# zxhuang1698/ShapeClipper

Measured on AMD Instinct MI355X. Metric: train-step images/sec (Pix3D cfg, bs32/GPU), higher is better.
Workload: dtype f32 (bf16x3-split MFMA, fp32 accumulate)

## Files before the change

### include/shapeclipper_hip.h

```cpp
#ifndef SHAPECLIPPER_HIP_H
#define SHAPECLIPPER_HIP_H
#include <stdint.h>
#ifdef __cplusplus
extern "C" {
#endif

int sc_chamfer3d_forward(const float* xyz1, const float* xyz2, float* dist1, float* dist2,
                         int32_t* idx1, int32_t* idx2, int b, int n, int m, void* stream);

int sc_chamfer3d_forward_split(const float* xyz1, const float* xyz2, float* dist1, float* dist2,
                               int32_t* idx1, int32_t* idx2, int b, int n, int m, int nsplit,
                               void* workspace, void* stream);

long long sc_chamfer3d_grid_workspace_bytes(int b, int n, int m);
int sc_chamfer3d_forward_grid(const float* xyz1, const float* xyz2, float* dist1, float* dist2,
                              int32_t* idx1, int32_t* idx2, int b, int n, int m, void* workspace, void* stream);

int sc_chamfer3d_backward(const float* xyz1, const float* xyz2, float* gradxyz1, float* gradxyz2,
                          const float* graddist1, const float* graddist2, const int32_t* idx1,
                          const int32_t* idx2, int b, int n, int m, void* stream);

long long sc_chamfer3d_backward_ordered_workspace_bytes(int b, int n, int m);
int sc_chamfer3d_backward_ordered_chunk(void);
int sc_chamfer3d_backward_ordered(const float* xyz1, const float* xyz2, float* gradxyz1, float* gradxyz2,
// ... 272 lines not shown

int sc_marching_cubes_mesh_vertex_blocks_per_image(int n_axis);
int sc_marching_cubes_mesh_vertex_count(const float* level, int n_images, int n_axis, float iso, int* block_counts, void* stream);
int sc_marching_cubes_mesh_vertex_scan(const int* block_counts, int n_images, int n_axis, long long* block_offsets, long long* per_image,
                                       void* stream);
int sc_marching_cubes_mesh_vertex_emit(const float* level, int n_images, int n_axis, float iso, const long long* block_offsets, float* verts,
                                       int* vmap, void* stream);
int sc_marching_cubes_mesh_face_emit(int n_images, int n_axis, const long long* block_offsets, const unsigned char* masks, const int* vmap,
                                     int* faces, void* stream);

int sc_camera_rays_forward(const float* pose, const float* intr, const long long* ray_idx, int n_images,
                           int rays_per_image, int image_width, float* cam_loc, float* ray_dirs, float* depth_fac,
                           void* stream);
int sc_camera_rays_backward(const float* pose, const float* intr, const long long* ray_idx, int n_images,
                            int rays_per_image, int image_width, const float* g_cam_loc, const float* g_ray_dirs,
                            const float* g_depth_fac, float* g_pose, float* g_intr, void* stream);

int sc_pose_from_trig_forward(const float* azim, const float* elev, const float* theta, const float* scale_focal,
                              const float* scale_dist, int n_images, float cam_dist, float focal, int image_width,
                              int image_height, float* pose, float* intr, void* stream);
int sc_pose_from_trig_backward(const float* azim, const float* elev, const float* theta, const float* scale_focal,
                               const float* scale_dist, int n_images, float cam_dist, float focal, int image_width,
                               int image_height, const float* g_pose, const float* g_intr, float* g_azim,
                               float* g_elev, float* g_theta, float* g_scale_focal, float* g_scale_dist, void* stream);

int sc_estimator_head_forward(const float* trig, const float* size_lin, const float* persp_lin, int n_rows,
                              float size_range, float persp_range, float* azim, float* elev, float* theta,
                              float* scale_focal, float* scale_dist, void* stream);
int sc_estimator_head_backward(const float* trig, const float* size_lin, const float* persp_lin, int n_rows,
                               float size_range, float persp_range, const float* const* grads, int n_groups,
                               float* g_trig, float* g_size_lin, float* g_persp_lin, void* stream);

int sc_camera_prior_max_images(void);
int sc_camera_prior_forward(const float* azim, const float* elev, const float* theta, const float* flip_azim,
                            const float* flip_elev, const float* flip_theta, int n_images, float elev_lo, float elev_hi,
                            float theta_lo, float theta_hi, float margin_eps, int emd_p, float* out, float* grads,
                            void* stream);
int sc_camera_prior_backward(const float* grads, int n_images, const float* G_margin, const float* G_uniform,
                             const float* G_sym, float* g_azim, float* g_elev, float* g_theta, float* g_flip_azim,
                             float* g_flip_elev, float* g_flip_theta, void* stream);

int sc_transform_normal_forward(const float* normals, const float* pose, int n_images, int n_per_image, float* out,
                                void* stream);
int sc_transform_normal_backward(const float* normals, const float* g_out, int n_images, int n_per_image, float* g_pose,
                                 void* stream);

int sc_loss_total_forward(const float* const* values, const float* weights, int n_terms, float* total, unsigned char* bad,
                          void* stream);
int sc_loss_total_backward(const float* weights, int n_terms, const float* G, float* g_values, void* stream);

long long sc_conv3x3_pack_floats(int cin, int cout, int hw);
long long sc_conv3x3_workspace_floats(int hw);
int sc_conv3x3_tile_channels(int hw);
int sc_conv3x3_pack_multi(const long long* table, int n, float* dst, long long total, void* stream);
int sc_conv3x3_pack_multi_units(const long long* table, int n, float* dst, long long total, void* stream);
int sc_conv3x3_pack(const float* w, float* w_pack, int cin, int cout, int hw, int transpose_flip, void* stream);
int sc_conv3x3_forward(const float* x, const float* w_pack, float* out, float* workspace, int batch, int cin, int cout, int hw,
                       void* stream);

long long sc_conv3x3_pack_floats_split(int cin, int cout, int hw);
long long sc_conv3x3_workspace_floats_split(int hw);
int sc_conv3x3_tile_channels_split(int hw);
int sc_conv3x3_forward_split(const float* x, const float* w_pack, float* out, float* workspace, int batch, int cin, int cout, int hw,
                             void* stream);
int sc_conv3x3_forward_add(const float* x, const float* w_pack, const float* addend, float* out, float* workspace, int batch, int cin,
                           int cout, int hw, int split, void* stream);

long long sc_conv3x3s2_bd_pack_floats(int cin, int cout, int hw);
long long sc_conv3x3s2_bd_workspace_floats(int hw);
int sc_conv3x3s2_bd_pack(const float* w, float* w_pack, int cin, int cout, int hw, void* stream);
int sc_conv3x3s2_backward_data(const float* gy, const float* w_pack, float* gx, float* workspace, int batch, int cin, int cout, int hw,
                               void* stream);
int sc_conv3x3s2_wgrad(const float* gy, const float* x, float* dw, float* workspace, int batch, int cin, int cout, int hw, void* stream);
long long sc_conv3x3s2_pack_floats(int cin, int cout, int hw);
long long sc_conv3x3s2_workspace_floats(int hw);
int sc_conv3x3s2_forward(const float* x, const float* w_pack, float* out, float* workspace, int batch, int cin, int cout, int hw,
                         void* stream);

long long sc_conv3x3_wgrad_workspace_floats(int cin, int cout);
int sc_conv3x3_wgrad(const float* gy, const float* x, float* dw, float* workspace, int batch, int cin, int cout, int hw, void* stream);
int sc_conv3x3_wgrad_split(const float* gy, const float* x, float* dw, float* workspace, int batch, int cin, int cout, int hw, void* stream);

long long sc_conv_stem_wgrad_workspace_floats(void);
int sc_conv_stem_forward(const float* x, const float* w, float* out, int batch, void* stream);
int sc_conv_stem_wgrad(const float* gy, const float* x, float* dw, float* workspace, int batch, void* stream);

long long sc_conv1x1s2_wgrad_workspace_floats(int cin, int cout);
int sc_conv1x1s2_forward(const float* x, const float* w, float* out, int batch, int cin, int cout, int hin, void* stream);
int sc_conv1x1s2_backward_data(const float* gy, const float* w, float* gx, int batch, int cin, int cout, int hin, void* stream);
int sc_conv1x1s2_wgrad(const float* gy, const float* x, float* dw, float* workspace, int batch, int cin, int cout, int hin, void* stream);

typedef struct sc_block_args {
    const float *x, *pf1, *pf2, *pb1, *pb2;
    const float *g1, *b1, *g2, *b2;
    float *rm1, *rv1, *rm2, *rv2;
    int64_t *nt1, *nt2;
    float *y1, *a1, *y2, *out, *st1, *st2;
    float *conv_ws, *bn_ws, *wgrad_ws;
    const float* d_out;
    float *dy2, *dres, *da1, *dy1, *dx, *gw1, *gw2, *dgb1, *dgb2;
    int batch, channels, hw, groups, training, split, need_dx;
    float mom1, eps1, mom2, eps2;
} sc_block_args;
int sc_basic_block_forward(const sc_block_args* args, void* stream);
int sc_basic_block_backward(const sc_block_args* args, void* stream);

int sc_linear_bn_supported(int N, int Cin, int Cout, int groups);
int sc_linear_bn_forward(const float* x, const float* w, const float* gamma, const float* beta, const float* res, float* y, float* out,
                         float* save_mean, float* save_rstd, float* run_mean, float* run_var, int64_t* n_tracked, int N, int Cin,
                         int Cout, int groups, int training, int relu, float eps, float momentum, void* stream);
int sc_linear_bn_backward(const float* g_out, const float* gy_next, const float* w_next, const float* g_add, int Cnext, const float* out,
                          const float* y, const float* save_mean, const float* save_rstd, const float* gamma, const float* x, float* gy,
                          float* g_res, float* dw, float* dgamma, float* dbeta, int N, int Cin, int Cout, int groups, int training, int relu,
                          void* stream);
int sc_linear_backward_data(const float* gy, const float* w, const float* g_add, float* dx, int N, int Cin, int Cout, void* stream);

int sc_latent_bias_forward(const float* z, const float* lat, const float* bias, const float* post, float* out, int B, int Z, int L, int NL,
                           void* stream);
int sc_latent_bias_backward(const float* g, const float* z, const float* lat, const float* post, float* g_z, float* g_lat, float* g_bias,
                            int B, int Z, int L, int NL, void* stream);

int sc_silhouette_distance(const float* masks, int n, int H, int W, float* dist, void* stream);
int sc_silhouette_rays(const float* dist, int n, int H, int W, int n_rays, double uniform_fac, const long long* seeds,
                       long long* ray_idx, void* stream);

int sc_clip_preprocess(const unsigned char* rgba, int n, int H, int W, int n_px, int bg, const int* h_bounds, const int* h_coef,
                       int h_taps, const int* v_bounds, const int* v_coef, int v_taps, unsigned char* tmp, float* out, void* stream);

int sc_vis_frames(const float* x, long long n_pixels, int channels, int kind, float lo, float scale, unsigned char* out, void* stream);

int sc_rgb_points_forward_split(const float* points, const float* grad, const float* feat, const float* v_pack,
                                const float* dbias, int n_points, int n_per_image, int n_images, int symmetric,
                                float* rgb, float* normal, void* stream);

long long sc_level_largest_component_scratch_bytes(int n_images, int n_axis);
int sc_level_largest_component(const float* level, int n_images, int n_axis, float iso, float* level_out, int32_t* n_components,
                               int32_t* inside_voxels, int32_t* kept_voxels, void* scratch, void* stream);

#define SC_SURFACE_HIT_MAX_RAYS (1 << 30)
int sc_ray_first_crossing(const float* z_vals, const float* sdf, int n_rays, int n_samples, float iso, float* t_lo, float* t_hi,
                          float* f_lo, float* f_hi, int32_t* hit, void* stream);
int sc_ray_bracket_step(const float* cam_loc, const float* ray_dirs, const float* f_new, const float* t_prev, int n_rays, float iso,
                        float* t_lo, float* t_hi, float* f_lo, float* f_hi, const int32_t* hit, float* t, float* points, void* stream);

int sc_set_reserved_cus(int n);
int sc_grid_cus(void);
int sc_conv3x3_release_tables(void);

#ifdef __cplusplus
}
#endif
#endif
```

### shapeclipper_amd/csrc/conv_stem.hip

```cpp
#include <hip/hip_runtime.h>

#include "grid_cus.hpp"
#include "shapeclipper_hip.h"

namespace sc {

typedef float st_f32x16 __attribute__((ext_vector_type(16)));

constexpr int ST_WI = 224, ST_WO = 112, ST_WP = 230, ST_K = 147, ST_KP = 148, ST_CO = 64;
constexpr int ST_HWI = ST_WI * ST_WI, ST_HWO = ST_WO * ST_WO;
constexpr int SF_PT = 256;
constexpr int SF_ROWS = 13;
constexpr int SF_CH = SF_ROWS * ST_WP;
constexpr int SF_PATCH = 3 * SF_CH;
constexpr int SF_WLD = 96;
constexpr int SF_LDS = ST_KP * SF_WLD + SF_PATCH;
constexpr int SF_NLOAD = (3 * SF_ROWS + 7) / 8;

__global__ __launch_bounds__(512, 1) void conv_stem_fwd_kernel(const float* __restrict__ x, const float* __restrict__ w,
                                                               float* __restrict__ out, int batch) {
    extern __shared__ float4 st_smem[];
    float* Ws = reinterpret_cast<float*>(st_smem);
    float* Xs = Ws + ST_KP * SF_WLD;
    const int tid = threadIdx.x, lane = tid & 63, wave = __builtin_amdgcn_readfirstlane(tid >> 6), half = lane >> 5;
    const int tiles = batch * (ST_HWO / SF_PT), G = gridDim.x, g = blockIdx.x;
    const int t_lo = (int)((long long)g * tiles / G), t_hi = (int)((long long)(g + 1) * tiles / G);

    for (int i = tid; i < ST_KP * SF_WLD; i += 512) {
        const int k = i / SF_WLD, co = i - k * SF_WLD;
        Ws[i] = (k < ST_K && co < ST_CO) ? w[co * ST_K + k] : 0.f;
    }

    float xv[SF_NLOAD][4];
    auto load = [&](int tile) {
        const int b = tile / (ST_HWO / SF_PT), p0 = (tile - b * (ST_HWO / SF_PT)) * SF_PT;
        const int r0 = 2 * (p0 / ST_WO) - 3;
        const float* xb = x + (size_t)b * 3 * ST_HWI;
#pragma unroll
        for (int l = 0; l < SF_NLOAD; ++l) {
            const int line = wave + 8 * l, ci = line / SF_ROWS, row = r0 + line - ci * SF_ROWS;
            const bool row_ok = line < 3 * SF_ROWS && row >= 0 && row < ST_WI;
#pragma unroll
            for (int c = 0; c < 4; ++c) {
                const int col = lane + 64 * c - 3;
                xv[l][c] = (row_ok && col >= 0 && col < ST_WI) ? xb[ci * ST_HWI + row * ST_WI + col] : 0.f;
            }
        }
    };
    auto store = [&]() {
#pragma unroll
        for (int l = 0; l < SF_NLOAD; ++l) {
            const int line = wave + 8 * l;
            if (line < 3 * SF_ROWS) {
#pragma unroll
                for (int c = 0; c < 4; ++c)
                    if (lane + 64 * c < ST_WP) Xs[line * ST_WP + lane + 64 * c] = xv[l][c];
            }
        }
    };

    if (t_lo < t_hi) load(t_lo);
    for (int tile = t_lo; tile < t_hi; ++tile) {
        __syncthreads();
        store();
        __syncthreads();
        if (tile + 1 < t_hi) load(tile + 1);
        const int b = tile / (ST_HWO / SF_PT), p0 = (tile - b * (ST_HWO / SF_PT)) * SF_PT;
        const int p = p0 + wave * 32 + (lane & 31), y = p / ST_WO, xo = p - y * ST_WO;
        const float* Bb = Xs + (y - p0 / ST_WO) * 2 * ST_WP + 2 * xo;
        const float* Ab = Ws + half * SF_WLD + (lane & 31);
        st_f32x16 acc[2];
#pragma unroll
        for (int r = 0; r < 16; ++r) acc[0][r] = acc[1][r] = 0.f;
#pragma unroll
        for (int j = 0; j < ST_KP / 2; ++j) {
            const int k0 = 2 * j, k1 = 2 * j + 1 < ST_K ? 2 * j + 1 : ST_K - 1;
            const int o0 = (k0 / 49) * SF_CH + ((k0 % 49) / 7) * ST_WP + k0 % 7, o1 = (k1 / 49) * SF_CH + ((k1 % 49) / 7) * ST_WP + k1 % 7;
            const float bv = Bb[o0 + half * (o1 - o0)];
            const float a0 = Ab[2 * j * SF_WLD], a1 = Ab[2 * j * SF_WLD + 32];
            acc[0] = __builtin_amdgcn_mfma_f32_32x32x2f32(a0, bv, acc[0], 0, 0, 0);
            acc[1] = __builtin_amdgcn_mfma_f32_32x32x2f32(a1, bv, acc[1], 0, 0, 0);
        }
        float* ob = out + (size_t)b * ST_CO * ST_HWO + p;
#pragma unroll
        for (int i = 0; i < 2; ++i)
#pragma unroll
            for (int r = 0; r < 16; ++r) ob[(size_t)(32 * i + (r & 3) + 8 * (r >> 2) + 4 * half) * ST_HWO] = acc[i][r];
    }
}

constexpr int SW_ROWS = 9;
constexpr int SW_CH = SW_ROWS * ST_WP;
constexpr int SW_PATCH = 3 * SW_CH;
constexpr int SW_ZERO = 1026;
static_assert((SW_PATCH + SW_ZERO) % 4 == 0, "the gy tile behind it is read with ds_read_b128");
constexpr int SW_GST = 2 * ST_WO + 4;
constexpr int SW_LDS = SW_PATCH + SW_ZERO + ST_CO * SW_GST;
constexpr int SW_PART = 2 * 5 * 16 * 64;

__global__ __launch_bounds__(512, 1) void conv_stem_wgrad_kernel(const float* __restrict__ gy, const float* __restrict__ x,
                                                                 float* __restrict__ partial, int batch) {
    extern __shared__ float4 st_smem[];
    float* Xs = reinterpret_cast<float*>(st_smem);
    float* Gs = Xs + SW_PATCH + SW_ZERO;
    const int tid = threadIdx.x, lane = tid & 63, wave = __builtin_amdgcn_readfirstlane(tid >> 6), half = lane >> 5;
    const int cot = wave & 1, kq = wave >> 1;
    const int steps = batch * (ST_WO / 2), G = gridDim.x, g = blockIdx.x;
    const int s_lo = (int)((long long)g * steps / G), s_hi = (int)((long long)(g + 1) * steps / G);

    for (int i = tid; i < SW_LDS; i += 512) Xs[i] = 0.f;

    float xv[4][4], gv[8][4];
    auto load = [&](int step) {
        const int b = step / (ST_WO / 2), y0 = 2 * (step - b * (ST_WO / 2));
        const float* xb = x + (size_t)b * 3 * ST_HWI;
#pragma unroll
        for (int l = 0; l < 4; ++l) {
            const int line = wave + 8 * l, ci = line / SW_ROWS, row = 2 * y0 - 3 + line - ci * SW_ROWS;
            const bool row_ok = line < 3 * SW_ROWS && row >= 0 && row < ST_WI;
#pragma unroll
            for (int c = 0; c < 4; ++c) {
                const int col = lane + 64 * c - 3;
                xv[l][c] = (row_ok && col >= 0 && col < ST_WI) ? xb[ci * ST_HWI + row * ST_WI + col] : 0.f;
            }
        }
        const float* gb = gy + ((size_t)b * ST_CO + 8 * wave) * ST_HWO + y0 * ST_WO;
#pragma unroll
        for (int ch = 0; ch < 8; ++ch)
#pragma unroll
            for (int c = 0; c < 4; ++c) gv[ch][c] = lane + 64 * c < 2 * ST_WO ? gb[ch * ST_HWO + lane + 64 * c] : 0.f;
    };
    auto store = [&]() {
#pragma unroll
        for (int l = 0; l < 4; ++l) {
            const int line = wave + 8 * l;
            if (line < 3 * SW_ROWS) {
#pragma unroll
                for (int c = 0; c < 4; ++c)
                    if (lane + 64 * c < ST_WP) Xs[line * ST_WP + lane + 64 * c] = xv[l][c];
            }
        }
#pragma unroll
        for (int ch = 0; ch < 8; ++ch)
#pragma unroll
            for (int c = 0; c < 4; ++c)
                if (lane + 64 * c < 2 * ST_WO) Gs[(8 * wave + ch) * SW_GST + lane + 64 * c] = gv[ch][c];
    };

    int tapb[5];
#pragma unroll
    for (int nt = 0; nt < 5; ++nt) {
        const int k = 32 * nt + (lane & 31);
        tapb[nt] = k < ST_K ? (k / 49) * SW_CH + ((k % 49) / 7) * ST_WP + k % 7 + 8 * half : SW_PATCH;
    }
    const float* Ab = Gs + (32 * cot + (lane & 31)) * SW_GST + 4 * half;

    st_f32x16 acc[5];
#pragma unroll
    for (int nt = 0; nt < 5; ++nt)
#pragma unroll
        for (int r = 0; r < 16; ++r) acc[nt][r] = 0.f;

    if (s_lo < s_hi) load(s_lo);
    __syncthreads();
    for (int step = s_lo; step < s_hi; ++step) {
        store();
        __syncthreads();
        if (step + 1 < s_hi) load(step + 1);
#pragma unroll
        for (int gi = 0; gi < 7; ++gi) {
            const int grp = 7 * kq + gi;
            const int r = grp / 14, x0 = (grp - 14 * r) * 8;
            const float4 a = *reinterpret_cast<const float4*>(Ab + r * ST_WO + x0);
            const int po = r * 2 * ST_WP + 2 * x0;
#pragma unroll
            for (int nt = 0; nt < 5; ++nt) {
                const float* bp = Xs + tapb[nt] + po;
#pragma unroll
                for (int s = 0; s < 4; ++s) {
                    const float av = s == 0 ? a.x : s == 1 ? a.y : s == 2 ? a.z : a.w;
                    acc[nt] = __builtin_amdgcn_mfma_f32_32x32x2f32(av, bp[2 * s], acc[nt], 0, 0, 0);
                }
            }
        }
        __syncthreads();
    }

    float* R = Gs;
#pragma unroll 1
    for (int q = 1; q < 4; ++q) {
        if (kq == q) {
#pragma unroll
            for (int nt = 0; nt < 5; ++nt)
#pragma unroll
                for (int r = 0; r < 16; ++r) R[((cot * 5 + nt) * 16 + r) * 64 + lane] = acc[nt][r];
        }
        __syncthreads();
        if (kq == 0) {
#pragma unroll
            for (int nt = 0; nt < 5; ++nt)
#pragma unroll
                for (int r = 0; r < 16; ++r) acc[nt][r] += R[((cot * 5 + nt) * 16 + r) * 64 + lane];
        }
        __syncthreads();
    }
    if (kq == 0) {
        float* dst = partial + (size_t)g * SW_PART;
#pragma unroll
        for (int nt = 0; nt < 5; ++nt)
#pragma unroll
            for (int r = 0; r < 16; ++r) dst[((cot * 5 + nt) * 16 + r) * 64 + lane] = acc[nt][r];
    }
}

__global__ void conv_stem_wgrad_reduce_kernel(const float* __restrict__ partial, float* __restrict__ dw, int G) {
    const int e = blockIdx.x * blockDim.x + threadIdx.x;
    if (e >= SW_PART) return;
    float s0 = 0.f, s1 = 0.f, s2 = 0.f, s3 = 0.f;
    int gi = 0;
    for (; gi + 3 < G; gi += 4) {
        s0 += partial[(size_t)gi * SW_PART + e];
        s1 += partial[(size_t)(gi + 1) * SW_PART + e];
        s2 += partial[(size_t)(gi + 2) * SW_PART + e];
        s3 += partial[(size_t)(gi + 3) * SW_PART + e];
    }
    for (; gi < G; ++gi) s0 += partial[(size_t)gi * SW_PART + e];
    const int lane = e & 63, r = (e >> 6) & 15, nt = (e >> 10) % 5, cot = e / (5 * 1024);
    const int co = 32 * cot + (r & 3) + 8 * (r >> 2) + 4 * (lane >> 5), k = 32 * nt + (lane & 31);
    if (k < ST_K) dw[co * ST_K + k] = (s0 + s1) + (s2 + s3);
}

static int stem_cus() { return grid_cus(); }

}

extern "C" long long sc_conv_stem_wgrad_workspace_floats(void) { return (long long)sc::stem_cus() * sc::SW_PART; }

extern "C" int sc_conv_stem_forward(const float* x, const float* w, float* out, int batch, void* stream) {
    if (batch <= 0) return (int)hipErrorInvalidValue;
    (void)hipFuncSetAttribute((const void*)sc::conv_stem_fwd_kernel, hipFuncAttributeMaxDynamicSharedMemorySize, sc::SF_LDS * 4);
    hipLaunchKernelGGL(sc::conv_stem_fwd_kernel, dim3(sc::stem_cus()), dim3(512), sc::SF_LDS * 4, (hipStream_t)stream, x, w, out, batch);
    return (int)hipGetLastError();
}

extern "C" int sc_conv_stem_wgrad(const float* gy, const float* x, float* dw, float* workspace, int batch, void* stream) {
    if (batch <= 0) return (int)hipErrorInvalidValue;
    const int G = sc::stem_cus();
    (void)hipFuncSetAttribute((const void*)sc::conv_stem_wgrad_kernel, hipFuncAttributeMaxDynamicSharedMemorySize, sc::SW_LDS * 4);
    hipLaunchKernelGGL(sc::conv_stem_wgrad_kernel, dim3(G), dim3(512), sc::SW_LDS * 4, (hipStream_t)stream, gy, x, workspace, batch);
    hipLaunchKernelGGL(sc::conv_stem_wgrad_reduce_kernel, dim3((sc::SW_PART + 255) / 256), dim3(256), 0, (hipStream_t)stream, workspace, dw, G);
    return (int)hipGetLastError();
}
```

### shapeclipper_amd/functional.py

```python
from __future__ import annotations

import torch

from . import ops


class SdfFunction(torch.autograd.Function):

    @staticmethod
    def forward(ctx, points, w_pack, cbias, n_per_image, symmetric, want_grad, want_feat, fused_backward=True):
        ctx.set_materialize_grads(False)
        points = points.contiguous()
        need = any(ctx.needs_input_grad[:3])
        res = ops.sdf_forward(points, w_pack, cbias, n_per_image, symmetric=symmetric, want_grad=want_grad,
                              want_feat=want_feat, stash=need)
        sdf, grad, feat = res[0], res[1], res[2]
        ctx.meta = (n_per_image, cbias.shape[0], symmetric, want_grad, want_feat)
        ctx.fused_backward = fused_backward
        if need:
            ctx.save_for_backward(points, w_pack, res[3], res[4] if want_grad else None)
        empty = points.new_empty(0)
        outs = (sdf, grad if want_grad else empty, feat if want_feat else empty)
        nd = [o for o, w in zip(outs[1:], (want_grad, want_feat)) if not w]
        if nd:
# ... 180 lines not shown
        return dx, dg, db, None, None, None, None, None, None, None


def _bn_fusable(bn, x):
    return (x.is_cuda and x.dtype == torch.float32 and x.dim() == 4 and bn.affine and bn.momentum is not None
            and (bn.training or bn.track_running_stats))


def bn_act(bn, x, residual=None, relu=True, groups=1):
    if not _bn_fusable(bn, x):
        out = bn(x) if groups == 1 else torch.cat([bn(c) for c in x.chunk(groups)], 0)
        if residual is not None:
            out = out + residual
        return torch.relu_(out) if relu else out
    training = bn.training or not bn.track_running_stats
    track = bn.track_running_stats
    return BnActFunction.apply(x, residual, bn.weight, bn.bias, bn.running_mean if track else None,
                               bn.running_var if track else None,
                               bn.num_batches_tracked if (track and training) else None,
                               training, float(bn.momentum), float(bn.eps), relu, groups)


def _bn_state(bn):
    training = bn.training or not bn.track_running_stats
    track = bn.track_running_stats
    return (bn.running_mean if track else None, bn.running_var if track else None,
            bn.num_batches_tracked if (track and training) else None, training, float(bn.momentum), float(bn.eps))


def bottleneck_linear(x, conv1, bn1, conv2, bn2, groups=1):
    C = x.shape[1]
    if not (x.is_cuda and x.dtype == torch.float32 and x.dim() == 2 and _bn_fusable(bn1, x[..., None, None]) and _bn_fusable(bn2, x[..., None, None])
            and conv1.bias is None and conv2.bias is None and conv1.weight.shape == (C, C, 1, 1) and conv2.weight.shape == (C, C, 1, 1)
            and x.shape[0] % groups == 0 and ops.linear_bn_supported(x.shape[0], C, C, groups)):
        return None
    if (bn1.training or bn2.training) and x.shape[0] // groups < 2:
        return None
    return BottleneckLinearFunction.apply(x, conv1.weight.view(C, C), bn1.weight, bn1.bias, conv2.weight.view(C, C), bn2.weight, bn2.bias,
                                          _bn_state(bn1), _bn_state(bn2), groups)


def bn_relu_maxpool(bn, x, groups=1):
    if not _bn_fusable(bn, x):
        out = bn(x) if groups == 1 else torch.cat([bn(c) for c in x.chunk(groups)], 0)
        return torch.nn.functional.max_pool2d(torch.relu_(out), 3, 2, 1)
    training = bn.training or not bn.track_running_stats
    track = bn.track_running_stats
    return BnReluPoolFunction.apply(x, bn.weight, bn.bias, bn.running_mean if track else None,
                                    bn.running_var if track else None,
                                    bn.num_batches_tracked if (track and training) else None,
                                    training, float(bn.momentum), float(bn.eps), groups)


class Conv3x3Function(torch.autograd.Function):

    @staticmethod
    def forward(ctx, x, w, pack_f, pack_b, split):
        x = ops._aligned(x)
        ctx.save_for_backward(x, w, pack_b)
        ctx.split = split
        if pack_f is None:
            pack_f = ops.conv3x3_pack(w, x.shape[2], False, split)
        return ops.conv3x3_apply(x, pack_f, w.shape[0], split)

    @staticmethod
    def backward(ctx, gy):
        x, w, pack_b = ctx.saved_tensors
        gy = ops._aligned(gy)
        gx = None
        if ctx.needs_input_grad[0]:
            gx = ops.conv3x3_apply(gy, pack_b if pack_b is not None else ops.conv3x3_pack(w, x.shape[2], True, ctx.split), w.shape[1], ctx.split)
        gw = None
        if ctx.needs_input_grad[1]:
            if ops.conv3x3_wgrad_supported(x.shape, w.shape):
                gw = ops.conv3x3_backward_weight(gy, x, split=ctx.split)
            else:
                gw = torch.ops.aten.convolution_backward(gy, x, w, None, [1, 1], [1, 1], [1, 1], False, [0, 0], 1, [False, True, False])[1]
        return gx, gw, None, None, None


class ConvStemFunction(torch.autograd.Function):

    @staticmethod
    def forward(ctx, x, w):
        x = ops._aligned(x)
        ctx.save_for_backward(x, w)
        return ops.conv_stem_forward(x, w)

    @staticmethod
    def backward(ctx, gy):
        x, w = ctx.saved_tensors
        gy = ops._aligned(gy)
        gx = None
        if ctx.needs_input_grad[0]:
            gx = torch.ops.aten.convolution_backward(gy, x, w, None, [2, 2], [3, 3], [1, 1], False, [0, 0], 1, [True, False, False])[0]
        gw = ops.conv_stem_backward_weight(gy, x) if ctx.needs_input_grad[1] else None
        return gx, gw


def conv_stem(conv, x):
    if (x.is_cuda and x.dtype == torch.float32 and conv.bias is None and conv.groups == 1 and conv.dilation == (1, 1)
            and ops.conv_stem_supported(x.shape, conv.weight.shape, conv.stride, conv.padding)):
        return ConvStemFunction.apply(x, conv.weight)
    return conv(x)


class Conv1x1S2Function(torch.autograd.Function):

    @staticmethod
    def forward(ctx, x, w):
        x = ops._aligned(x)
        ctx.save_for_backward(x, w)
        return ops.conv1x1s2_forward(x, w)

    @staticmethod
    def backward(ctx, gy):
        x, w = ctx.saved_tensors
        gy = ops._aligned(gy)
        gx = ops.conv1x1s2_backward_data(gy, w) if ctx.needs_input_grad[0] else None
        gw = ops.conv1x1s2_backward_weight(gy, x) if ctx.needs_input_grad[1] else None
        return gx, gw


def conv1x1s2(conv, x):
    if (x.is_cuda and x.dtype == torch.float32 and conv.bias is None and conv.groups == 1 and conv.dilation == (1, 1)
            and ops.conv1x1s2_supported(x.shape, conv.weight.shape, conv.stride, conv.padding)):
        return Conv1x1S2Function.apply(x, conv.weight)
    return conv(x)


class Conv3x3S2Function(torch.autograd.Function):

    @staticmethod
    def forward(ctx, x, w):
        x = ops._aligned(x)
        ctx.save_for_backward(x, w)
        return ops.conv3x3s2_forward(x, w)

    @staticmethod
    def backward(ctx, gy):
        x, w = ctx.saved_tensors
        gy = ops._aligned(gy)
        from .model import resnet
        if resnet.HIP_CONV3X3_S2_GRADS and ops.conv3x3s2_grads_supported(x.shape, w.shape):
            gx = gw = None
            if ctx.needs_input_grad[0]:
                if resnet.HIP_CONV3X3_SPLIT:
                    gx = ops.conv3x3s2_backward_data(gy, w, x.shape[2])
                else:
                    gx = torch.ops.aten.convolution_backward(gy, x, w, None, [2, 2], [1, 1], [1, 1], False, [0, 0], 1, [True, False, False])[0]
            if ctx.needs_input_grad[1]:
                gw = ops.conv3x3s2_backward_weight(gy, x)
            return gx, gw
        gx, gw, _ = torch.ops.aten.convolution_backward(gy, x, w, None, [2, 2], [1, 1], [1, 1], False, [0, 0], 1,
                                                        [ctx.needs_input_grad[0], ctx.needs_input_grad[1], False])
        return gx, gw


def conv3x3s2(conv, x):
    if (x.is_cuda and x.dtype == torch.float32 and conv.bias is None and conv.groups == 1 and conv.dilation == (1, 1)
            and ops.conv3x3s2_supported(x.shape, conv.weight.shape, conv.stride, conv.padding)):
        return Conv3x3S2Function.apply(x, conv.weight)
    return conv(x)


def conv3x3_takes(conv, x):
    return (x.is_cuda and x.dtype == torch.float32 and conv.bias is None and conv.groups == 1 and conv.dilation == (1, 1)
            and ops.conv3x3_supported(x.shape, conv.weight.shape, conv.stride, conv.padding))


def conv3x3(conv, x, packs=None):
    if not conv3x3_takes(conv, x):
        return conv(x)
    if packs is not None and id(conv.weight) in packs.index:
        return Conv3x3Function.apply(x, conv.weight, packs.get(conv.weight, 0), packs.get(conv.weight, 1), packs.split)
    from .model import resnet
    return Conv3x3Function.apply(x, conv.weight, None, None, bool(resnet.HIP_CONV3X3_SPLIT))


class BasicBlockFunction(torch.autograd.Function):

    @staticmethod
    def forward(ctx, x, w1, g1, b1, w2, g2, b2, pf1, pb1, pf2, pb2, split, bn1_state, bn2_state, groups):
        x = ops._aligned(x)
        out, saved = ops.basic_block_forward(x, pf1, pf2, g1, b1, g2, b2, bn1_state, bn2_state, split, groups)
        ctx.meta = (split, bn1_state[3], groups)
# ... 157 lines not shown
```

### shapeclipper_amd/ops.py

```python
from __future__ import annotations

import collections
import ctypes
import weakref

import torch

from . import _lib
from .packing import n_tiles

_SCRATCH = {}


def _scratch(tag, dev, n_floats):
    if dev.type != "cuda":
        raise RuntimeError(_lib.NO_CPU)
    key = (tag, dev.index, torch._C._cuda_getCurrentRawStream(dev.index))
    buf = _SCRATCH.get(key)
    if buf is None or buf.numel() < n_floats:
        buf = _SCRATCH[key] = torch.empty(n_floats, device=dev, dtype=torch.float32)
    return buf


SDF_SCRATCH_FLOATS = 256 * 8 * 5 * 1024
# ... 902 lines not shown
def conv3x3_backward_data(gy, w, split=False):
    return _conv3x3(gy, w, True, split)


def conv3x3_wgrad_supported(x_shape, w_shape, stride=1, padding=1) -> bool:
    return conv3x3_supported(x_shape, w_shape, stride, padding) and w_shape[0] % 64 == 0 and w_shape[1] % 64 == 0


def conv3x3_backward_weight(gy, x, split=False):
    lib = _lib.load()
    gy, x = _aligned(gy), _aligned(x)
    B, cout, H, _ = gy.shape
    cin = x.shape[1]
    n = lib.sc_conv3x3_wgrad_workspace_floats(cin, cout)
    if n < 0 or H not in CONV3X3_SIDES or x.shape[0] != B or tuple(x.shape[2:]) != (H, H):
        raise RuntimeError("shapeclipper_amd: sc_conv3x3_wgrad does not take gy %s with x %s" % (tuple(gy.shape), tuple(x.shape)))
    ws = _scratch("conv wgrad", x.device, n)
    dw = torch.empty(cout, cin, 3, 3, device=x.device, dtype=torch.float32)
    fn = lib.sc_conv3x3_wgrad_split if split else lib.sc_conv3x3_wgrad
    _lib.check(fn(_lib.ptr(gy), _lib.ptr(x), _lib.ptr(dw), _lib.ptr(ws), B, cin, cout, H, _lib.stream()), "sc_conv3x3_wgrad")
    return dw


class BlockArgs(ctypes.Structure):
    _fields_ = ([(n, ctypes.c_void_p) for n in ("x", "pf1", "pf2", "pb1", "pb2", "g1", "b1", "g2", "b2", "rm1", "rv1", "rm2", "rv2", "nt1", "nt2",
                                   "y1", "a1", "y2", "out", "st1", "st2", "conv_ws", "bn_ws", "wgrad_ws", "d_out",
                                   "dy2", "dres", "da1", "dy1", "dx", "gw1", "gw2", "dgb1", "dgb2")]
                + [(n, ctypes.c_int) for n in ("batch", "channels", "hw", "groups", "training", "split", "need_dx")]
                + [(n, ctypes.c_float) for n in ("mom1", "eps1", "mom2", "eps2")])


def _wgrad_workspace(x, cin, cout):
    return _scratch("conv wgrad", x.device, _lib.load().sc_conv3x3_wgrad_workspace_floats(cin, cout))


def basic_block_forward(x, pf1, pf2, g1, b1, g2, b2, bn1_state, bn2_state, split, groups):
    B, C, H, _ = x.shape
    rm1, rv1, nt1, training, mom1, eps1 = bn1_state
    rm2, rv2, nt2, _, mom2, eps2 = bn2_state
    y1, a1, y2, out = (torch.empty_like(x) for _ in range(4))
    st = torch.empty(2, 2, groups, C, device=x.device, dtype=torch.float32)
    a = BlockArgs()
    a.x, a.pf1, a.pf2 = x.data_ptr(), pf1.data_ptr(), pf2.data_ptr()
    a.g1, a.b1, a.g2, a.b2 = g1.data_ptr(), b1.data_ptr(), g2.data_ptr(), b2.data_ptr()
    a.rm1, a.rv1, a.nt1, a.rm2, a.rv2, a.nt2 = _p(rm1), _p(rv1), _p(nt1), _p(rm2), _p(rv2), _p(nt2)
    a.y1, a.a1, a.y2, a.out = y1.data_ptr(), a1.data_ptr(), y2.data_ptr(), out.data_ptr()
    a.st1, a.st2 = st[0].data_ptr(), st[1].data_ptr()
    a.conv_ws, a.bn_ws = _conv_workspace(x.device, H, split).data_ptr(), _bn_partial(x, groups)
    a.batch, a.channels, a.hw, a.groups, a.training, a.split = B, C, H, groups, 1 if training else 0, 1 if split else 0
    a.mom1, a.eps1, a.mom2, a.eps2 = mom1, eps1, mom2, eps2
    code = _lib.load().sc_basic_block_forward(ctypes.byref(a), _lib.raw_stream(x.get_device()))
    if code:
        _lib.check(code, "sc_basic_block_forward")
    return out, (y1, a1, y2, st[0], st[1])


def basic_block_backward(d_out, x, saved, out, pb1, pb2, g1, b1, g2, b2, training, split, groups, need_dx, need_w1, need_w2):
    y1, a1, y2, st1, st2 = saved
    B, C, H, _ = x.shape
    dy2, da1, dy1 = (torch.empty_like(x) for _ in range(3))
    dx, dres = (torch.empty_like(x), torch.empty_like(x)) if need_dx else (None, None)
    gw1 = torch.empty(C, C, 3, 3, device=x.device, dtype=torch.float32) if need_w1 else None
    gw2 = torch.empty(C, C, 3, 3, device=x.device, dtype=torch.float32) if need_w2 else None
    dgb = torch.empty(2, 2, C, device=x.device, dtype=torch.float32)
    a = BlockArgs()
    a.x, a.pb1, a.pb2, a.d_out = x.data_ptr(), pb1.data_ptr(), pb2.data_ptr(), d_out.data_ptr()
    a.g1, a.b1, a.g2, a.b2 = g1.data_ptr(), b1.data_ptr(), g2.data_ptr(), b2.data_ptr()
    a.y1, a.a1, a.y2, a.out, a.st1, a.st2 = y1.data_ptr(), a1.data_ptr(), y2.data_ptr(), out.data_ptr(), st1.data_ptr(), st2.data_ptr()
    a.dy2, a.da1, a.dy1, a.dres, a.dx = dy2.data_ptr(), da1.data_ptr(), dy1.data_ptr(), _p(dres), _p(dx)
    a.gw1, a.gw2, a.dgb1, a.dgb2 = _p(gw1), _p(gw2), dgb[0].data_ptr(), dgb[1].data_ptr()
    a.conv_ws, a.bn_ws = _conv_workspace(x.device, H, split).data_ptr(), _bn_partial(x, groups)
    a.wgrad_ws = _wgrad_workspace(x, C, C).data_ptr() if (need_w1 or need_w2) else None
    a.batch, a.channels, a.hw, a.groups, a.training, a.split, a.need_dx = B, C, H, groups, 1 if training else 0, 1 if split else 0, 1 if need_dx else 0
    code = _lib.load().sc_basic_block_backward(ctypes.byref(a), _lib.raw_stream(x.get_device()))
    if code:
        _lib.check(code, "sc_basic_block_backward")
    return dx, gw1, dgb[0, 0], dgb[0, 1], gw2, dgb[1, 0], dgb[1, 1]


def conv_stem_supported(x_shape, w_shape, stride=2, padding=3) -> bool:
    return (tuple(x_shape[1:]) == (3, 224, 224) and tuple(w_shape) == (64, 3, 7, 7) and stride in (2, (2, 2)) and padding in (3, (3, 3)))


def conv_stem_forward(x, w):
    lib = _lib.load()
    x, w = _aligned(x), _aligned(w)
    out = torch.empty(x.shape[0], 64, 112, 112, device=x.device, dtype=torch.float32)
    _lib.check(lib.sc_conv_stem_forward(_lib.ptr(x), _lib.ptr(w), _lib.ptr(out), x.shape[0], _lib.stream()), "sc_conv_stem_forward")
    return out


def conv_stem_backward_weight(gy, x):
    lib = _lib.load()
    gy, x = _aligned(gy), _aligned(x)
    ws = _scratch("conv stem", x.device, lib.sc_conv_stem_wgrad_workspace_floats())
    dw = torch.empty(64, 3, 7, 7, device=x.device, dtype=torch.float32)
    _lib.check(lib.sc_conv_stem_wgrad(_lib.ptr(gy), _lib.ptr(x), _lib.ptr(dw), _lib.ptr(ws), x.shape[0], _lib.stream()), "sc_conv_stem_wgrad")
    return dw


def conv1x1s2_supported(x_shape, w_shape, stride=2, padding=0) -> bool:
    return (len(x_shape) == 4 and tuple(w_shape[2:]) == (1, 1) and stride in (2, (2, 2)) and padding in (0, (0, 0)) and x_shape[2] == x_shape[3]
            and x_shape[2] % 2 == 0 and w_shape[1] == x_shape[1] and w_shape[0] % 64 == 0 and w_shape[1] % 64 == 0)


def conv1x1s2_forward(x, w):
    lib = _lib.load()
    x, w = _aligned(x), _aligned(w)
    B, cin, H, _ = x.shape
    out = torch.empty(B, w.shape[0], H // 2, H // 2, device=x.device, dtype=torch.float32)
    _lib.check(lib.sc_conv1x1s2_forward(_lib.ptr(x), _lib.ptr(w), _lib.ptr(out), B, cin, w.shape[0], H, _lib.stream()), "sc_conv1x1s2_forward")
    return out


def conv1x1s2_backward_data(gy, w):
    lib = _lib.load()
    gy, w = _aligned(gy), _aligned(w)
    B, cout, Ho, _ = gy.shape
    gx = torch.empty(B, w.shape[1], 2 * Ho, 2 * Ho, device=gy.device, dtype=torch.float32)
    _lib.check(lib.sc_conv1x1s2_backward_data(_lib.ptr(gy), _lib.ptr(w), _lib.ptr(gx), B, w.shape[1], cout, 2 * Ho, _lib.stream()),
               "sc_conv1x1s2_backward_data")
    return gx


def conv1x1s2_backward_weight(gy, x):
    lib = _lib.load()
    gy, x = _aligned(gy), _aligned(x)
    B, cin, H, _ = x.shape
    cout = gy.shape[1]
    n = lib.sc_conv1x1s2_wgrad_workspace_floats(cin, cout)
    ws = _scratch("conv 1x1s2", x.device, n)
    dw = torch.empty(cout, cin, 1, 1, device=x.device, dtype=torch.float32)
    _lib.check(lib.sc_conv1x1s2_wgrad(_lib.ptr(gy), _lib.ptr(x), _lib.ptr(dw), _lib.ptr(ws), B, cin, cout, H, _lib.stream()), "sc_conv1x1s2_wgrad")
    return dw


def conv3x3s2_supported(x_shape, w_shape, stride=2, padding=1) -> bool:
    return (len(x_shape) == 4 and tuple(w_shape[2:]) == (3, 3) and stride in (2, (2, 2)) and padding in (1, (1, 1)) and x_shape[2] == x_shape[3]
            and x_shape[2] in (56, 28, 14) and w_shape[1] == x_shape[1] and w_shape[0] % 8 == 0 and w_shape[1] % 8 == 0)


def conv3x3s2_forward(x, w):
    lib = _lib.load()
    x, w = _aligned(x), _aligned(w)
    B, cin, H, _ = x.shape
    cout = w.shape[0]
    n = lib.sc_conv3x3s2_pack_floats(cin, cout, H)
    if n < 0:
        raise RuntimeError("shapeclipper_amd: sc_conv3x3s2 does not take [%d, %d, %d, %d] * %s" % (B, cin, H, H, tuple(w.shape)))
    w_pack = torch.empty(n, device=x.device, dtype=torch.float32)
    _lib.check(lib.sc_conv3x3_pack(_lib.ptr(w), _lib.ptr(w_pack), cin, cout, H, 4, _lib.stream()), "sc_conv3x3_pack")
    ws = _scratch("conv s2 %d" % H, x.device, lib.sc_conv3x3s2_workspace_floats(H))
    out = torch.empty(B, cout, H // 2, H // 2, device=x.device, dtype=torch.float32)
    _lib.check(lib.sc_conv3x3s2_forward(_lib.ptr(x), _lib.ptr(w_pack), _lib.ptr(out), _lib.ptr(ws), B, cin, cout, H, _lib.stream()),
               "sc_conv3x3s2_forward")
    return out


def conv3x3s2_grads_supported(x_shape, w_shape) -> bool:
    return conv3x3s2_supported(x_shape, w_shape) and w_shape[0] % 64 == 0 and w_shape[1] % 64 == 0


def conv3x3s2_backward_data(gy, w, hw):
    lib = _lib.load()
    gy, w = _aligned(gy), _aligned(w)
    B, cout = gy.shape[0], gy.shape[1]
    cin = w.shape[1]
    n = lib.sc_conv3x3s2_bd_pack_floats(cin, cout, hw)
    if n < 0 or tuple(gy.shape[2:]) != (hw // 2, hw // 2) or w.shape[0] != cout:
        raise RuntimeError("shapeclipper_amd: sc_conv3x3s2_backward_data does not take gy %s with w %s" % (tuple(gy.shape), tuple(w.shape)))
    w_pack = torch.empty(n, device=gy.device, dtype=torch.float32)
# ... 237 lines not shown
```

Baseline: 984.1.

## Add bf16x3-split MFMA path for the 7x7 stem conv forward

Adds a stem forward kernel that splits the weights and input patch into three bf16 pieces in LDS and accumulates six cross-term products with 32x32x16 bf16 MFMA instead of 32x32x2 f32 MFMA. The 147-long reduction is regrouped into 11 kernel-row slices of 8 taps, with double-buffered operand reads and scheduling barriers. This is meant to cut the stem's MFMA instruction count while keeping near-fp32 accuracy. It costs the extra split arithmetic when staging tiles and wastes some MMA work on zero-padded taps. The path is chosen by the existing HIP_CONV3X3_SPLIT flag.

```diff
diff --git a/include/shapeclipper_hip.h b/include/shapeclipper_hip.h
--- a/include/shapeclipper_hip.h
+++ b/include/shapeclipper_hip.h
@@ -378,7 +378,7 @@
 int sc_conv3x3_wgrad_split(const float* gy, const float* x, float* dw, float* workspace, int batch, int cin, int cout, int hw, void* stream);
 
 long long sc_conv_stem_wgrad_workspace_floats(void);
-int sc_conv_stem_forward(const float* x, const float* w, float* out, int batch, void* stream);
+int sc_conv_stem_forward(const float* x, const float* w, float* out, int batch, int split, void* stream);
 int sc_conv_stem_wgrad(const float* gy, const float* x, float* dw, float* workspace, int batch, void* stream);
 
 long long sc_conv1x1s2_wgrad_workspace_floats(int cin, int cout);
diff --git a/shapeclipper_amd/csrc/conv_stem.hip b/shapeclipper_amd/csrc/conv_stem.hip
--- a/shapeclipper_amd/csrc/conv_stem.hip
+++ b/shapeclipper_amd/csrc/conv_stem.hip
@@ -80,6 +80,147 @@
             const float a0 = Ab[2 * j * SF_WLD], a1 = Ab[2 * j * SF_WLD + 32];
             acc[0] = __builtin_amdgcn_mfma_f32_32x32x2f32(a0, bv, acc[0], 0, 0, 0);
             acc[1] = __builtin_amdgcn_mfma_f32_32x32x2f32(a1, bv, acc[1], 0, 0, 0);
+        }
+        float* ob = out + (size_t)b * ST_CO * ST_HWO + p;
+#pragma unroll
+        for (int i = 0; i < 2; ++i)
+#pragma unroll
+            for (int r = 0; r < 16; ++r) ob[(size_t)(32 * i + (r & 3) + 8 * (r >> 2) + 4 * half) * ST_HWO] = acc[i][r];
+    }
+}
+
+typedef __bf16 st_bf16x8 __attribute__((ext_vector_type(8)));
+typedef __bf16 st_bf16x2 __attribute__((ext_vector_type(2)));
+typedef unsigned st_u32x4 __attribute__((ext_vector_type(4)));
+
+constexpr int SS_KS = 11;
+constexpr int SS_WHALF = SS_KS * ST_CO;
+constexpr int SS_WPIECE = 2 * SS_WHALF * 4;
+constexpr int SS_XROW = ST_WP / 2;
+constexpr int SS_LINES = 3 * SF_ROWS;
+constexpr int SS_XPIECE = (SS_LINES + 1) * SS_XROW;
+constexpr int SS_LDS = 3 * (SS_WPIECE + SS_XPIECE);
+static_assert(ST_WP % 2 == 0 && SS_XPIECE % 4 == 0 && SS_WPIECE % 4 == 0, "piece planes stay 16-byte aligned");
+
+__device__ __forceinline__ void st_split(float v, __bf16& h0, __bf16& h1, __bf16& h2) {
+    h0 = (__bf16)v;
+    const float r1 = v - (float)h0;
+    h1 = (__bf16)r1;
+    const float r2 = r1 - (float)h1;
+    h2 = (__bf16)r2;
+}
+
+__global__ __launch_bounds__(512, 1) void conv_stem_fwd_split_kernel(const float* __restrict__ x, const float* __restrict__ w,
+                                                                     float* __restrict__ out, int batch) {
+    extern __shared__ float4 st_smem[];
+    unsigned* Xs = reinterpret_cast<unsigned*>(st_smem);
+    st_u32x4* Wq = reinterpret_cast<st_u32x4*>(Xs + 3 * SS_XPIECE);
+    const int tid = threadIdx.x, lane = tid & 63, wave = __builtin_amdgcn_readfirstlane(tid >> 6), half = lane >> 5;
+    const int tiles = batch * (ST_HWO / SF_PT), G = gridDim.x, g = blockIdx.x;
+    const int t_lo = (int)((long long)g * tiles / G), t_hi = (int)((long long)(g + 1) * tiles / G);
+
+    for (int v = tid; v < SS_KS * 2 * ST_CO; v += 512) {
+        const int co = v & (ST_CO - 1), ks = (v / ST_CO) % SS_KS, h = v / (ST_CO * SS_KS);
+        const int ci = ks < 7 ? h : 2, ky = ks < 7 ? ks : 2 * (ks - 7) + h;
+        st_bf16x8 p0, p1, p2;
+#pragma unroll
+        for (int s = 0; s < 8; ++s) {
+            const float f = (ky < 7 && s < 7) ? w[co * ST_K + ci * 49 + ky * 7 + s] : 0.f;
+            __bf16 h0, h1, h2;
+            st_split(f, h0, h1, h2);
+            p0[s] = h0, p1[s] = h1, p2[s] = h2;
+        }
+        st_u32x4* d = Wq + h * (3 * SS_WHALF) + ks * ST_CO + co;
+        d[0] = __builtin_bit_cast(st_u32x4, p0);
+        d[SS_WHALF] = __builtin_bit_cast(st_u32x4, p1);
+        d[2 * SS_WHALF] = __builtin_bit_cast(st_u32x4, p2);
+    }
+    for (int i = tid; i < 3 * SS_XROW; i += 512) Xs[(i / SS_XROW) * SS_XPIECE + SS_LINES * SS_XROW + i % SS_XROW] = 0u;
+
+    float xv[SF_NLOAD][4];
+    auto load = [&](int tile) {
+        const int b = tile / (ST_HWO / SF_PT), p0 = (tile - b * (ST_HWO / SF_PT)) * SF_PT;
+        const int r0 = 2 * (p0 / ST_WO) - 3;
+        const float* xb = x + (size_t)b * 3 * ST_HWI;
+#pragma unroll
+        for (int l = 0; l < SF_NLOAD; ++l) {
+            const int line = wave + 8 * l, ci = line / SF_ROWS, row = r0 + line - ci * SF_ROWS;
+            const bool row_ok = line < SS_LINES && row >= 0 && row < ST_WI;
+#pragma unroll
+            for (int c = 0; c < 4; ++c) {
+                const int col = 2 * (lane + 64 * (c >> 1)) + (c & 1) - 3;
+                xv[l][c] = (row_ok && col >= 0 && col < ST_WI) ? xb[ci * ST_HWI + row * ST_WI + col] : 0.f;
+            }
+        }
+    };
+    auto store = [&]() {
+#pragma unroll
+        for (int l = 0; l < SF_NLOAD; ++l) {
+            const int line = wave + 8 * l;
+            if (line < SS_LINES) {
+#pragma unroll
+                for (int c = 0; c < 2; ++c) {
+                    st_bf16x2 q0, q1, q2;
+#pragma unroll
+                    for (int e = 0; e < 2; ++e) {
+                        __bf16 h0, h1, h2;
+                        st_split(xv[l][2 * c + e], h0, h1, h2);
+                        q0[e] = h0, q1[e] = h1, q2[e] = h2;
+                    }
+                    if (lane + 64 * c < SS_XROW) {
+                        unsigned* d = Xs + line * SS_XROW + lane + 64 * c;
+                        d[0] = __builtin_bit_cast(unsigned, q0);
+                        d[SS_XPIECE] = __builtin_bit_cast(unsigned, q1);
+                        d[2 * SS_XPIECE] = __builtin_bit_cast(unsigned, q2);
+                    }
+                }
+            }
+        }
+    };
+
+    if (t_lo < t_hi) load(t_lo);
+    for (int tile = t_lo; tile < t_hi; ++tile) {
+        __syncthreads();
+        store();
+        __syncthreads();
+        if (tile + 1 < t_hi) load(tile + 1);
+        const int b = tile / (ST_HWO / SF_PT), p0 = (tile - b * (ST_HWO / SF_PT)) * SF_PT;
+        const int p = p0 + wave * 32 + (lane & 31), y = p / ST_WO, xo = p - y * ST_WO;
+        const unsigned* Bb = Xs + (y - p0 / ST_WO) * 2 * SS_XROW + xo;
+        const unsigned* Bb1 = Bb + half * SF_ROWS * SS_XROW;
+        const unsigned* Bb2 = Bb + half * SS_XROW;
+        const st_u32x4* Ab = Wq + half * (3 * SS_WHALF) + (lane & 31);
+        st_f32x16 acc[2];
+#pragma unroll
+        for (int r = 0; r < 16; ++r) acc[0][r] = acc[1][r] = 0.f;
+        st_u32x4 a[2][2][3], bq[2][3];
+        auto read_ops = [&](int ks, int set) {
+            const unsigned* bp = ks < 7 ? Bb1 + ks * SS_XROW : Bb2 + (2 * SF_ROWS + 2 * (ks - 7)) * SS_XROW;
+#pragma unroll
+            for (int q = 0; q < 3; ++q) {
+                bq[set][q] = st_u32x4{bp[q * SS_XPIECE], bp[q * SS_XPIECE + 1], bp[q * SS_XPIECE + 2], bp[q * SS_XPIECE + 3]};
+                a[set][0][q] = Ab[q * SS_WHALF + ks * ST_CO];
+                a[set][1][q] = Ab[q * SS_WHALF + ks * ST_CO + 32];
+            }
+        };
+        read_ops(0, 0);
+#pragma unroll
+        for (int ks = 0; ks < SS_KS; ++ks) {
+            const int c = ks & 1;
+            if (ks + 1 < SS_KS) read_ops(ks + 1, c ^ 1);
+            __builtin_amdgcn_sched_barrier(0);
+#pragma unroll
+            for (int term = 0; term < 6; ++term) {
+                constexpr int PA[6] = {0, 2, 1, 0, 1, 0}, PB[6] = {2, 0, 1, 1, 0, 0};
+#pragma unroll
+                for (int i = 0; i < 2; ++i)
+                    acc[i] = __builtin_amdgcn_mfma_f32_32x32x16_bf16(__builtin_bit_cast(st_bf16x8, a[c][i][PA[term]]),
+                                                                     __builtin_bit_cast(st_bf16x8, bq[c][PB[term]]), acc[i], 0, 0, 0);
+            }
+            asm volatile("" : "+v"(acc[0]), "+v"(acc[1])
+                         : "v"(a[c][0][0]), "v"(a[c][0][1]), "v"(a[c][0][2]), "v"(a[c][1][0]), "v"(a[c][1][1]), "v"(a[c][1][2]), "v"(bq[c][0]),
+                           "v"(bq[c][1]), "v"(bq[c][2]));
+            __builtin_amdgcn_sched_barrier(0);
         }
         float* ob = out + (size_t)b * ST_CO * ST_HWO + p;
 #pragma unroll
@@ -236,8 +377,13 @@
 
 extern "C" long long sc_conv_stem_wgrad_workspace_floats(void) { return (long long)sc::stem_cus() * sc::SW_PART; }
 
-extern "C" int sc_conv_stem_forward(const float* x, const float* w, float* out, int batch, void* stream) {
+extern "C" int sc_conv_stem_forward(const float* x, const float* w, float* out, int batch, int split, void* stream) {
     if (batch <= 0) return (int)hipErrorInvalidValue;
+    if (split) {
+        (void)hipFuncSetAttribute((const void*)sc::conv_stem_fwd_split_kernel, hipFuncAttributeMaxDynamicSharedMemorySize, sc::SS_LDS * 4);
+        hipLaunchKernelGGL(sc::conv_stem_fwd_split_kernel, dim3(sc::stem_cus()), dim3(512), sc::SS_LDS * 4, (hipStream_t)stream, x, w, out, batch);
+        return (int)hipGetLastError();
+    }
     (void)hipFuncSetAttribute((const void*)sc::conv_stem_fwd_kernel, hipFuncAttributeMaxDynamicSharedMemorySize, sc::SF_LDS * 4);
     hipLaunchKernelGGL(sc::conv_stem_fwd_kernel, dim3(sc::stem_cus()), dim3(512), sc::SF_LDS * 4, (hipStream_t)stream, x, w, out, batch);
     return (int)hipGetLastError();
diff --git a/shapeclipper_amd/functional.py b/shapeclipper_amd/functional.py
--- a/shapeclipper_amd/functional.py
+++ b/shapeclipper_amd/functional.py
@@ -286,10 +286,10 @@
 class ConvStemFunction(torch.autograd.Function):
 
     @staticmethod
-    def forward(ctx, x, w):
+    def forward(ctx, x, w, split=False):
         x = ops._aligned(x)
         ctx.save_for_backward(x, w)
-        return ops.conv_stem_forward(x, w)
+        return ops.conv_stem_forward(x, w, split=split)
 
     @staticmethod
     def backward(ctx, gy):
@@ -299,13 +299,14 @@
         if ctx.needs_input_grad[0]:
             gx = torch.ops.aten.convolution_backward(gy, x, w, None, [2, 2], [3, 3], [1, 1], False, [0, 0], 1, [True, False, False])[0]
         gw = ops.conv_stem_backward_weight(gy, x) if ctx.needs_input_grad[1] else None
-        return gx, gw
+        return gx, gw, None
 
 
 def conv_stem(conv, x):
     if (x.is_cuda and x.dtype == torch.float32 and conv.bias is None and conv.groups == 1 and conv.dilation == (1, 1)
             and ops.conv_stem_supported(x.shape, conv.weight.shape, conv.stride, conv.padding)):
-        return ConvStemFunction.apply(x, conv.weight)
+        from .model import resnet
+        return ConvStemFunction.apply(x, conv.weight, bool(resnet.HIP_CONV3X3_SPLIT))
     return conv(x)
 
 
diff --git a/shapeclipper_amd/ops.py b/shapeclipper_amd/ops.py
--- a/shapeclipper_amd/ops.py
+++ b/shapeclipper_amd/ops.py
@@ -1008,11 +1008,11 @@
     return (tuple(x_shape[1:]) == (3, 224, 224) and tuple(w_shape) == (64, 3, 7, 7) and stride in (2, (2, 2)) and padding in (3, (3, 3)))
 
 
-def conv_stem_forward(x, w):
+def conv_stem_forward(x, w, split=False):
     lib = _lib.load()
     x, w = _aligned(x), _aligned(w)
     out = torch.empty(x.shape[0], 64, 112, 112, device=x.device, dtype=torch.float32)
-    _lib.check(lib.sc_conv_stem_forward(_lib.ptr(x), _lib.ptr(w), _lib.ptr(out), x.shape[0], _lib.stream()), "sc_conv_stem_forward")
+    _lib.check(lib.sc_conv_stem_forward(_lib.ptr(x), _lib.ptr(w), _lib.ptr(out), x.shape[0], int(bool(split)), _lib.stream()), "sc_conv_stem_forward")
     return out
 
 
```

Result: slower. 974.1 (-1.0%).
